# jjery2243542/adaptive_voice_conversion

Hardware: AMD Instinct MI355X
Metric: mel-segments/sec (80x128) train step (higher is better)
Workload: dtype f32; 1 GPU; BASELINE configs[1]: recon+KL train step (fwd, loss, bwd, clip, Adam-amsgrad), 80-mel x 128-frame segments, batch 256/GPU, fp32; global_batch=256, parallelism=dp1, world_size=1

## Files before the change

adaptive_voice_conversion_amd/_lib.py:

```python
import ctypes
import os

_HERE = os.path.dirname(os.path.abspath(__file__))
LIB_PATH = os.path.join(_HERE, "csrc", "libavc_hip.so")
_lib = None

MAX_BLOCKS = 8
PLAN_INFERENCE, PLAN_SPEAKER_ONLY = 1, 2
GRADS_ALL, GRADS_DECODER, GRADS_ENCODERS, GRADS_SPEAKER, GRADS_CONTENT = 0, 1, 2, 3, 4


class EncoderCfg(ctypes.Structure):
    _fields_ = [(n, ctypes.c_int) for n in ("c_in", "c_h", "c_out", "kernel_size", "bank_size", "bank_scale", "c_bank",
                                            "n_conv_blocks", "n_dense_blocks")] + [("subsample", ctypes.c_int * MAX_BLOCKS), ("act", ctypes.c_int)]


class DecoderCfg(ctypes.Structure):
    _fields_ = [(n, ctypes.c_int) for n in ("c_in", "c_cond", "c_h", "c_out", "kernel_size", "n_conv_blocks")] + \
               [("upsample", ctypes.c_int * MAX_BLOCKS), ("act", ctypes.c_int)]


class ModelCfg(ctypes.Structure):
    _fields_ = [("spk", EncoderCfg), ("enc", EncoderCfg), ("dec", DecoderCfg)]


class ReluSite(ctypes.Structure):
    _fields_ = [(n, ctypes.c_int) for n in ("kind", "B", "C", "T")] + \
               [(n, ctypes.c_long) for n in ("act_off", "sb", "sc", "st", "y_off", "stat_off", "cond_off", "cond_sb", "storage")]


class Tuning(ctypes.Structure):
    _fields_ = [(n, ctypes.c_int) for n in ("struct_size", "single_stream", "dec_split_min", "conv_x3", "wgrad_x3", "dgrad_par", "bank_switch",
                                            "conv_ck5", "wgrad_batch", "wgrad_batch_wgs", "wgrad_target_wgs", "conv_ablation", "wgrad_ablation",
                                            "op_compute_dtype", "side_prio", "tile12_wgs")] + \
               [(n, ctypes.c_long) for n in ("wgrad_batch_units", "tile_thr11", "tile_thr21", "ck16_wgs", "ck32_wgs", "kg_wgs", "conv_min_lds", "in_pairs_nv", "bh_ck5", "wgrad_cw8", "dec_wgrad_flush", "dec_wgrad_wgs", "conv_walk", "conv_walk_min", "conv_in_fuse", "dbg_streams")]


PLAN_X3 = 4
PLAN_RAGGED = 8
PLAN_BF16S = 16
PLAN_CONTENT_ONLY, PLAN_DECODER_ONLY, PLAN_PART_GRADS = 32, 64, 128
PLAN_INPUT_GRADS = 256
FWD_WEIGHTS_PACKED = 1
PLAN_EMB_INPUT = 512
ERR_PAIR_SHAPE = -12
c_void_p, c_long, c_int, c_float = ctypes.c_void_p, ctypes.c_long, ctypes.c_int, ctypes.c_float


def make_tuning(lib, overrides=None):
    t = Tuning()
# ... 140 lines not shown
```

adaptive_voice_conversion_amd/csrc/avc_common.h:

```cpp
#pragma once
#include <stdint.h>

#define AVC_MAX_GROUPS 8
#define AVC_THREADS 256

typedef float f32x16 __attribute__((ext_vector_type(16)));
typedef float f32x4 __attribute__((ext_vector_type(4)));
typedef short avc_s16x4 __attribute__((ext_vector_type(4)));

enum {
    AVC_COMPUTE_F32 = 0,
    AVC_COMPUTE_BF16 = 1,
    AVC_COMPUTE_F32X3 = 2,
    AVC_COMPUTE_BF16S = 3,
};

enum {
    AVC_RES_NONE = 0,
    AVC_RES_IDENTITY = 1,
    AVC_RES_AVGPOOL2 = 2,
    AVC_RES_POOLT = 3,
    AVC_RES_UPT = 4,
    AVC_RES_UP2 = 5,
};
// ... 94 lines not shown

struct WgradArgs {
    ConvSrc x;
    ConvSrc dy;
    int B, Cin, Cout, Tin, Tout;
    int KS, padL, stride;
    int chunks_per_sample, total_chunks, Tc, spc;
    int bf16;
    int tiles;
    int grp;
    int grid;
    int chunk_cost;
    int slots;
    int tNB, tWCO, tCW;
    int cw8;
    int rows_per_src;
    long cost_begin;
    long cost_total;
    long slab_need, dbslab_need;
    float* slab;
    float* dbslab;
    float* dw;
    float* db;
    long dw_src_stride, db_src_stride;
};
#define AVC_WGRAD_MAXL 16
struct WgradBatch {
    int nlayers;
    int dbg;
    int lds_floats;
// ... 202 lines not shown
```

adaptive_voice_conversion_amd/csrc/avc_internal.h:

```cpp
#pragma once
#include <string.h>

#include "avc_common.h"
#include "avc_hip.h"

struct PackArgs {
    const float* src[12];
    int nsrc, rows_per_src;
    int Cout, Cin, KS;
    int dgrad, CK, nchunk, M, Mp;
    float* dst;
    int img;
    int mb;
};

const avc_tuning& avc_default_tuning();
avc_tuning& avc_op_tuning();
long avc_pack_total(const PackArgs& p);

int avc_conv_ck(const avc_tuning& tun, int KS);
int avc_conv_pick_tile(const avc_tuning& tun, int Mp, int B, int Tout, int ngroups, int Kred);
long avc_conv_num_wgs(int tile, int Mp, int B, int Tout, int ngroups);
int avc_conv_ck_for(const avc_tuning& tun, int KS, long wgs, int mode, int stride, int Tout, int tile);
int avc_launch_conv(const ConvArgs& a, hipStream_t stream, int force_tile, const avc_tuning& tun);
// ... 13 lines not shown
int avc_launch_dsp_mag(const float* spec, int F, int T, float* mag, hipStream_t s);
int avc_launch_dsp_db_norm(const float* in, int C, int T, float ref_db, float max_db, float* out, hipStream_t s);
int avc_launch_dsp_denorm_amp(const float* in, int C, int T, float ref_db, float max_db, float* out, hipStream_t s);
int avc_launch_dsp_preemph(const float* y, long L, float a, float* out, hipStream_t s);
int avc_launch_dsp_deemph(const float* x, long L, float a, float* out, hipStream_t s);
int avc_launch_dsp_frame_power(const float* y, long L, int frame_length, int hop, int n_frames, float* out, hipStream_t s);
#define AVC_PACK_BATCH 16
int avc_launch_pack_batch(const PackArgs* ps, int n, hipStream_t stream);
#define AVC_PACK_PIECE 2048
#define AVC_PACK_STAGE 8192
int avc_pack_stage_rows(const PackArgs& p);
long avc_pack_pieces(const PackArgs& p);
int avc_launch_pack_table(const PackArgs* dev_tab, const void* dev_blk, int nblk, double bytes, const float* params, float* ws, hipStream_t stream);

void avc_wgrad_geometry(WgradArgs& a);
void avc_wgrad_plan_batch(WgradArgs* layers, int n, int target_wgs);
int avc_launch_wgrad_batch(const WgradArgs* layers, int n, hipStream_t stream, int ablation = 0);

int avc_launch_in_fwd(const INFwdArgs& a, hipStream_t s);
int avc_launch_in_bwd(const INBwdArgs& a, hipStream_t s);
int avc_launch_in_fwd_pairs(const INFwdArgs& a, hipStream_t s);
int avc_launch_in_bwd_pairs(const INBwdArgs& a, hipStream_t s);
int avc_launch_to_pairs(const float* x, long sxb, long sxc, long sxt, int B, int C, int T, float* dst, long db, long dc, hipStream_t s);
int avc_launch_reparam_fwd_pairs(const float* muls, const float* eps, int B, int C, int Tb, float* z, hipStream_t s);
int avc_launch_timepool_fwd_pairs(const float* in, int B, int C, int T, float* out, hipStream_t s);
int avc_launch_timepool_bwd_pairs(const float* dP, const float* amask, int B, int C, int T, float* G, float* dy, float slope, hipStream_t s);
int avc_launch_rag_in_fwd(const RagINArgs& a, hipStream_t s);
int avc_launch_rag_copy_rows(const float* x, long xsc, long xst, const int* T, const int* off, int B, int M, int sumT, float* dst, int CC, int c0,
                             hipStream_t s);
int avc_launch_rag_timepool_fwd(const float* in, const int* T, const int* off, int B, int C, float* out, hipStream_t s);
// ... 47 lines not shown
```

adaptive_voice_conversion_amd/csrc/conv_wgrad.hip:

```cpp
#include <hip/hip_runtime.h>
#include <stdlib.h>
#include <string.h>
#include <type_traits>
#include <vector>

#include "avc_common.h"
#include "avc_internal.h"
#include "conv_x3_shared.h"
#include "bf16_pairs.h"

static constexpr __host__ __device__ int wg_dyrow(bool lin) { return lin ? 36 : 33; }
static constexpr __host__ __device__ int wg_xrow_lin(int KS) {
    int r = (31 + KS + 3) / 4;
    return 4 * (r | 1);
}
#define WG_THREADS 512
static constexpr __host__ __device__ int wg_threads(int CW) { return (CW + 4) * 64; }

static constexpr __host__ __device__ int wg_group(int BF, int NB) { return BF == 2 ? (NB >= 4 ? 2 : 4) : 1; }
static constexpr __host__ __device__ int wg_stages(int BF, int NB) { return 2 * wg_group(BF, NB); }
#ifndef AVC_WGRAD_BHX_WAVES
#define AVC_WGRAD_BHX_WAVES 3
#endif

// ... 46 lines not shown
        const int cc = a.chunk_cost;
        s.layer = layer;
        s.tile = (int)(g / a.total_chunks);
        s.c_begin = (int)(g - (long)s.tile * a.total_chunks);
        const long tile_last = (long)(s.tile + 1) * a.total_chunks;
        s.c_end = (int)((g_end < tile_last ? g_end : tile_last) - (long)s.tile * a.total_chunks);
        g += s.c_end - s.c_begin;
        const long cs = a.cost_begin + (long)s.tile * a.total_chunks * cc;
        const int w_first = (int)((cs * G) / Ctot), w_last = (int)(((cs + (long)(a.total_chunks - 1) * cc) * G) / Ctot);
        s.nsplit = w_last - w_first + 1;
        s.z = w - w_first;
        return true;
    }
};

template <int KS, bool RT, int NB, int WCO, bool LIN, int BF, int CW = 4>
struct WgCfg {
    static constexpr int WCI = CW / WCO;
    static constexpr int TCO = 32 * WCO;
    static constexpr int TCI = 32 * NB * WCI;
    static constexpr int NACC = KS * NB;
    static constexpr bool BH = BF == 2;
    static constexpr int RCO = BH ? TCO / 2 : TCO, RCI = BH ? TCI / 2 : TCI;
    static constexpr int WG_DYROW = wg_dyrow(LIN);
    static constexpr int NPD = (RCO * WG_DYROW + 255) / 256;
    static constexpr int NPX = (RCI * (LIN ? wg_xrow_lin(KS) : (KS == 1 ? 33 : 71)) + 255) / 256;
    static constexpr int TPR = 256 / RCO;
    static constexpr int CPT = 32 / TPR;
    static constexpr int NBROW = BH ? 16 : 32;
    static constexpr int GRP = wg_group(BF, NB);
    static constexpr int NSTG = wg_stages(BF, NB);
    static constexpr bool BHX = BH && LIN && !RT;
    static constexpr int ROW16 = 40;
    static constexpr int ND16 = (RCO * 10 + 63) / 64, NX16 = (RCI * 10 + 63) / 64;
    static constexpr int NPD16 = (ND16 + 3) / 4, NPX16 = (NX16 + 3) / 4;
};
static __device__ __forceinline__ bool wg_wide16(const WgradArgs& a) {
    return (a.Tout & 31) == 0 && a.Tin == a.Tout && a.spc == 1 && a.x.st == 1 && a.dy.st == 1 && a.x.ps == 1 && a.dy.ps == 1 &&
           ((a.x.sc | a.x.sb | a.dy.sc | a.dy.sb) & 3) == 0 && ((((unsigned long)a.x.ptr) | ((unsigned long)a.dy.ptr)) & 15) == 0;
}

template <int KS, bool RT, int NB, int WCO, bool LIN, int BF, int CW>
static __device__ __forceinline__ void wg_producer(const WgradBatch& bt, float* smem, int tid, int lane, int wave) {
    using C = WgCfg<KS, RT, NB, WCO, LIN, BF, CW>;
    constexpr int TCO = C::TCO, TCI = C::TCI, RCO = C::RCO, RCI = C::RCI, WG_DYROW = C::WG_DYROW, NPD = C::NPD, NPX = C::NPX, TPR = C::TPR, CPT = C::CPT;
    constexpr int NSTG = C::NSTG, GRP = C::GRP;
    constexpr bool BH = C::BH;
    const int dbg = bt.dbg;
    const int ptid = tid & 255;
    unsigned dyo[NPD], xo[NPX];
    int xq[NPX];
    WgSegIter it(bt);
    WgSeg sg;
    while (it.next(bt, sg)) {
        const WgradArgs& a = bt.L[sg.layer];
        const int KSr = RT ? a.KS : KS;
        const int ci_tiles = avc_cdiv(a.Cin, TCI);
        const int CoutR = BH ? a.Cout >> 1 : a.Cout, CinR = BH ? a.Cin >> 1 : a.Cin;
        const float* xptr = a.x.ptr;
        const float* dyptr = a.dy.ptr;
        const int Tc = a.Tc, spc = a.spc;
        const int lgTc = 31 - __builtin_clz(Tc);
        const int XSEG = (Tc - 1) * a.stride + KSr;
        const int XROW = LIN ? wg_xrow_lin(KSr) : ((spc * XSEG) | 1);
        const bool wide = C::BHX && wg_wide16(a);
        const int DYROWW = wide ? C::ROW16 : WG_DYROW;
        const int DYS = wide ? RCO * C::ROW16 : RCO * WG_DYROW, XS = wide ? RCI * C::ROW16 : RCI * XROW;
        const int DYSP = wide ? (DYS + 255) & ~255 : (DYS + 63) & ~63, XSP = wide ? (XS + 255) & ~255 : (XS + 63) & ~63;
        float* dyT = smem;
        float* xT = smem + NSTG * DYSP;
        const float inv_xrow = 1.0f / (float)XROW;
        const int tile = sg.tile, c_begin = sg.c_begin, c_end = sg.c_end;
        const int co0 = (tile / ci_tiles) * TCO, ci0 = (tile % ci_tiles) * TCI;
        const int co0r = BH ? co0 >> 1 : co0, ci0r = BH ? ci0 >> 1 : ci0;
        const bool do_db = (a.db != nullptr) && (ci0 == 0);
        float dbsum = 0.f, dbsum1 = 0.f;
        const bool fastm = !wide && (spc > 1) && (a.Tout == Tc) && (a.B % spc == 0) && (XSP <= NPX * 256);
        const bool fastp = wide || fastm || ((spc == 1) && (a.Tout % 32 == 0) && (XSP <= NPX * 256));
        unsigned dyo16[C::BHX ? C::NPD16 : 1], xo16[C::BHX ? C::NPX16 : 1];
        int xedge[C::BHX ? C::NPX16 : 1];
        if constexpr (C::BHX) {
            if (wide) {
#pragma unroll
                for (int i = 0; i < C::NPD16; ++i) {
                    const int f = (wave + 4 * i) * 64 + lane;
                    int row = f / 10;
                    const int pc = f - row * 10;
                    row = row < RCO ? row : RCO - 1;
                    int co = co0r + row;
                    co = co < CoutR ? co : CoutR - 1;
                    dyo16[i] = 4u * (unsigned)((long)co * a.dy.sc + 4 * (pc < 8 ? pc : 0));
                }
#pragma unroll
                for (int i = 0; i < C::NPX16; ++i) {
                    const int f = (wave + 4 * i) * 64 + lane;
                    int row = f / 10;
                    const int pc = f - row * 10;
                    row = row < RCI ? row : RCI - 1;
                    int ci = ci0r + row;
                    ci = ci < CinR ? ci : CinR - 1;
                    xo16[i] = 4u * (unsigned)((long)ci * a.x.sc + 4 * pc);
                    xedge[i] = pc == 0 ? 1 : (pc == 9 ? -1 : 0);
                }
            }
        }
        auto issue16 = [&](int chunk, int buf) {
            if constexpr (C::BHX) {
                const int cb = chunk / a.chunks_per_sample;
                const int t0 = (chunk - cb * a.chunks_per_sample) * 32;
                const float* dyb = dyptr + ((long)cb * a.dy.sb + t0);
                const float* xb = xptr + ((long)cb * a.x.sb + t0) - 4;
                const bool first = t0 == 0, last = t0 + 32 == a.Tout;
                float* dd = dyT + buf * DYSP;
                float* xd = xT + buf * XSP;
#pragma unroll
                for (int i = 0; i < C::NPD16; ++i)
                    if (wave + 4 * i < C::ND16) avc_glds16_s(dyb, dyo16[i], dd + (wave + 4 * i) * 256);
#pragma unroll
                for (int i = 0; i < C::NPX16; ++i)
                    if (wave + 4 * i < C::NX16) {
                        unsigned v = xo16[i];
                        if (first && xedge[i] > 0) v += 16u;
                        if (last && xedge[i] < 0) v -= 16u;
                        avc_glds16_s(xb, v, xd + (wave + 4 * i) * 256);
                    }
            }
// ... 174 lines not shown
                    a.db[(long)(co / rows) * a.db_src_stride + co % rows] = v0;
                    a.db[(long)((co + 1) / rows) * a.db_src_stride + (co + 1) % rows] = v1;
                }
            } else {
                const int co = co0 + ptid / TPR;
                if (co < a.Cout) a.db[(long)(co / rows) * a.db_src_stride + co % rows] = v0;
            }
        };
        if (do_db) {
#pragma unroll
            for (int o = 1; o < TPR; o <<= 1) {
                dbsum += __shfl_xor(dbsum, o);
                if (BH) dbsum1 += __shfl_xor(dbsum1, o);
            }
        }
        if (dbg & 8) continue;
        if (sg.nsplit == 1) {
            if (do_db) store_db(dbsum, dbsum1);
            continue;
        }
        float* dbs_t = do_db ? a.dbslab + ((long)(tile / ci_tiles) * a.slots) * TCO : nullptr;
        if (do_db && (ptid % TPR) == 0) {
            if constexpr (BH) {
                dbs_t[(long)sg.z * TCO + 2 * (ptid / TPR)] = dbsum;
                dbs_t[(long)sg.z * TCO + 2 * (ptid / TPR) + 1] = dbsum1;
            } else {
                dbs_t[(long)sg.z * TCO + ptid / TPR] = dbsum;
            }
        }
    }
}

template <int KS, bool RT, int NB, int WCO, bool LIN, int BF, bool X3, int CW>
static __device__ __forceinline__ void wg_consumer(const WgradBatch& bt, float* smem, int tid, int lane, int wave) {
    using C = WgCfg<KS, RT, NB, WCO, LIN, BF, CW>;
    constexpr int WCI = C::WCI, TCO = C::TCO, TCI = C::TCI, NACC = C::NACC, RCO = C::RCO, RCI = C::RCI, WG_DYROW = C::WG_DYROW, NBROW = C::NBROW;
    constexpr int NSTG = C::NSTG;
    constexpr bool BH = C::BH;
    const int dbg = bt.dbg;
    const int wave_m = wave / WCI, wave_n = wave % WCI, li = lane & 31, h = lane >> 5;
    f32x16 acc[NACC];
    WgSegIter it(bt);
    WgSeg sg;
    while (it.next(bt, sg)) {
        const WgradArgs& a = bt.L[sg.layer];
        const int KSr = RT ? a.KS : KS;
        const int ci_tiles = avc_cdiv(a.Cin, TCI);
        const int Tc = a.Tc, spc = a.spc;
        const int lgTc = 31 - __builtin_clz(Tc);
        const int XSEG = (Tc - 1) * a.stride + KSr;
        const int XROW = LIN ? wg_xrow_lin(KSr) : ((spc * XSEG) | 1);
        const bool wide = C::BHX && wg_wide16(a);
        const int DYS = wide ? RCO * C::ROW16 : RCO * WG_DYROW, XS = wide ? RCI * C::ROW16 : RCI * XROW;
        const int DYSP = wide ? (DYS + 255) & ~255 : (DYS + 63) & ~63, XSP = wide ? (XS + 255) & ~255 : (XS + 63) & ~63;
        const float* dyT = smem;
        const float* xT = smem + NSTG * DYSP;
        int tcs = wide ? sg.c_begin % a.chunks_per_sample : 0;
        const long tile_floats = (long)CW * KSr * NB * 1024;
        const int tile = sg.tile, c_begin = sg.c_begin, c_end = sg.c_end;
        const int co0 = (tile / ci_tiles) * TCO, ci0 = (tile % ci_tiles) * TCI;
#pragma unroll
        for (int j = 0; j < NACC; ++j)
#pragma unroll
            for (int r = 0; r < 16; ++r) acc[j][r] = 0.f;
        __syncthreads();
        __syncthreads();
        auto chunk_loop = [&](auto wtag) {
        constexpr bool WIDE = decltype(wtag)::value;
        constexpr int GRP = C::GRP;
        for (int chunk = c_begin; chunk < c_end; ++chunk) {
            const int rel = chunk - c_begin;
            const int buf = GRP == 1 ? (rel & 1) : ((rel / GRP) & 1) * GRP + rel % GRP;
            const bool first_c = tcs == 0, last_c = tcs == a.chunks_per_sample - 1;
            if (WIDE && ++tcs == a.chunks_per_sample) tcs = 0;
            if (!(dbg & 2)) {
                const float* arow = dyT + buf * DYSP + (BH ? (wave_m * 32 + li) >> 1 : wave_m * 32 + li) * (WIDE ? C::ROW16 : WG_DYROW);
                const float* brow = xT + buf * XSP + (BH ? (wave_n * NB * 32 + li) >> 1 : wave_n * NB * 32 + li) * (WIDE ? C::ROW16 : XROW);
                auto body = [&](auto ktag) {
                    constexpr int K = decltype(ktag)::value;
                    auto tap_on = [&](int j) { return !RT || j < KSr; };
                    const float* arow_h = arow + h;
                    const float* brow_h = brow + h;
                    auto ldfrag = [&](int s, float& av, float (&bv)[NB * K]) {
                        const float* bp;
                        if constexpr (LIN) {
                            av = arow_h[2 * s];
                            bp = brow_h + 2 * s;
                        } else {
                            const int qcol = 2 * s + h;
                            const int sl = qcol >> lgTc, tl = qcol & (Tc - 1);
                            av = arow[qcol];
                            bp = brow + sl * XSEG + tl * a.stride;
// ... 11 lines not shown
                                constexpr int PADL = K / 2, PADR = (K & 1) ? K / 2 : K / 2 - 1;
                                constexpr int P0 = (4 - PADL) / 4, P1 = (11 + PADR) / 4;
                                auto fetchw = [&](int kb, unsigned (&ad)[8], unsigned (&xr)[NB][16]) {
                                    const float* ap = arow + 16 * kb + 8 * h;
                                    const float* bp = brow + 16 * kb + 8 * h;
#pragma unroll
                                    for (int i4 = 0; i4 < 2; ++i4) {
                                        const f32x4 v = *(const f32x4*)(ap + 4 * i4);
#pragma unroll
                                        for (int i = 0; i < 4; ++i) ad[4 * i4 + i] = bh_as_u32(v[i]);
                                    }
#pragma unroll
                                    for (int nb = 0; nb < NB; ++nb)
#pragma unroll
                                        for (int i4 = P0; i4 <= P1; ++i4) {
                                            const f32x4 v = *(const f32x4*)(bp + nb * NBROW * C::ROW16 + 4 * i4);
#pragma unroll
                                            for (int i = 0; i < 4; ++i) xr[nb][4 * i4 + i] = bh_as_u32(v[i]);
                                        }
                                };
                                auto blockw = [&](int kb, const unsigned (&ad)[8], unsigned (&xr)[NB][16]) {
                                    if (PADL > 0 && first_c && kb == 0) {
#pragma unroll
                                        for (int nb = 0; nb < NB; ++nb)
#pragma unroll
                                            for (int i = 1; i <= PADL; ++i) xr[nb][4 - i] = h == 0 ? xr[nb][4 + i] : xr[nb][4 - i];
                                    }
                                    if (PADR > 0 && last_c && kb == 1) {
#pragma unroll
                                        for (int nb = 0; nb < NB; ++nb)
#pragma unroll
// ... 128 lines not shown
                                    f32x16& c = acc[nb * KS + j];
                                    c = avc_mfma_bf16x8(at[2], q0, c);
                                    c = avc_mfma_bf16x8(at[0], q2, c);
                                    c = avc_mfma_bf16x8(at[1], q1, c);
                                    c = avc_mfma_bf16x8(at[1], q0, c);
                                    c = avc_mfma_bf16x8(at[0], q1, c);
                                    c = avc_mfma_bf16x8(at[0], q0, c);
                                }
                            }
                        };
                        float a0[8], x0[NB][NX], a1[8], x1[NB][NX];
                        fetch(0, a0, x0);
                        fetch(1, a1, x1);
                        block(a0, x0);
                        block(a1, x1);
                    } else if constexpr (LIN) {
                        constexpr int NX4 = (K + 6) / 4;
                        auto ldgrp = [&](int gq, f32x4& av, f32x4 (&xv)[NB][NX4]) {
                            const int c = 8 * gq + 4 * h;
                            av = *(const f32x4*)(arow + c);
#pragma unroll
                            for (int nb = 0; nb < NB; ++nb)
#pragma unroll
                                for (int i4 = 0; i4 < NX4; ++i4)
                                    if (!RT || 4 * i4 < 3 + KSr) xv[nb][i4] = *(const f32x4*)(brow + nb * 32 * XROW + c + 4 * i4);
                        };
                        f32x4 av[2], xv[2][NB][NX4];
                        ldgrp(0, av[0], xv[0]);
#pragma unroll
                        for (int gq = 0; gq < 4; ++gq) {
                            const int cur = gq & 1;
                            if (gq + 1 < 4) ldgrp(gq + 1, av[cur ^ 1], xv[cur ^ 1]);
                            __builtin_amdgcn_sched_barrier(0);
                            if constexpr (BF != 0) {
                                const avc_s16x4 ap = avc_pack_bf16x4(av[cur][0], av[cur][1], av[cur][2], av[cur][3]);
#pragma unroll
                                for (int nb = 0; nb < NB; ++nb)
#pragma unroll
                                    for (int j = 0; j < K; ++j) {
                                        if (!tap_on(j)) continue;
// ... 46 lines not shown
#pragma unroll
                            for (int nb = 0; nb < NB; ++nb)
#pragma unroll
                                for (int j = 0; j < K; ++j)
                                    if (tap_on(j)) acc[nb * KS + j] = __builtin_amdgcn_mfma_f32_32x32x2f32(av[cur], bv[cur][nb * K + j], acc[nb * KS + j], 0, 0, 0);
                            __builtin_amdgcn_sched_barrier(0);
                        }
                    }
                };
                static_assert(!RT || KS == 8, "run-time tap counts are built for up to 8 taps");
                body(KTag<KS>{});
            }
            if (!(dbg & 4) && (GRP == 1 || rel % GRP == GRP - 1 || chunk + 1 == c_end)) __syncthreads();
        }
        };
        if constexpr (C::BHX) {
            if (wide) chunk_loop(std::true_type{});
            else chunk_loop(std::false_type{});
        } else {
            chunk_loop(std::false_type{});
        }

        auto store_final = [&]() {
            const int rows = a.rows_per_src;
#pragma unroll
            for (int nb = 0; nb < NB; ++nb) {
                const int ci = ci0 + (wave_n * NB + nb) * 32 + li;
#pragma unroll
                for (int r = 0; r < 16; ++r) {
                    const int co = co0 + wave_m * 32 + (r & 3) + 8 * (r >> 2) + 4 * h;
                    if (co < a.Cout && ci < a.Cin) {
// ... 63 lines not shown

struct WgradKey {
    int KST, rt, NB, WCO, CW, lin;
    bool operator==(const WgradKey& o) const { return KST == o.KST && rt == o.rt && NB == o.NB && WCO == o.WCO && CW == o.CW && lin == o.lin; }
};
static size_t wgrad_lds_bytes_for(const WgradArgs& a, int NB, int WCO, int CW) {
    const int half = a.bf16 == AVC_COMPUTE_BF16S ? 2 : 1;
    const int TCO = 32 * WCO / half, TCI = 32 * NB * (CW / WCO) / half;
    const int XSEG = (a.Tc - 1) * a.stride + a.KS;
    const bool lin = a.Tc == 32 && a.stride == 1;
    const int XROW = lin ? wg_xrow_lin(a.KS) : ((a.spc * XSEG) | 1), WG_DYROW = wg_dyrow(lin);
    size_t stage = (size_t)((TCO * WG_DYROW + 63) & ~63) + ((TCI * XROW + 63) & ~63);
    if (half == 2 && lin) {
        const size_t s16 = (size_t)((TCO * 40 + 255) & ~255) + ((TCI * 40 + 255) & ~255);
        stage = s16 > stage ? s16 : stage;
    }
    return (size_t)wg_stages(half == 2 ? 2 : 0, NB) * stage * 4 + 64;
}
static WgradKey wgrad_key(const WgradArgs& a) {
    WgradKey k;
    wgrad_shape(a, &k.NB, &k.WCO, &k.CW);
    if (a.KS == 1 && k.NB == 4 && wgrad_lds_bytes_for(a, 4, 4, 4) > 158 * 1024) {
        k.NB = 1;
        k.WCO = 2;
    }
    if (k.CW == 8 && wgrad_lds_bytes_for(a, k.NB, k.WCO, 8) > 158 * 1024) {
        k.CW = 4;
        k.WCO = 2;
    }
    if (a.KS == 1) { k.KST = 1; k.rt = 0; }
    else if (a.KS == 5 && (k.WCO == 2 || k.CW == 8)) { k.KST = 5; k.rt = 0; }
    else { k.KST = 8; k.rt = 1; }
    k.lin = (a.Tc == 32 && a.stride == 1) ? 1 : 0;
    return k;
}

void avc_wgrad_geometry(WgradArgs& a) {
    if (a.Tout >= 32) {
        a.Tc = 32;
        a.spc = 1;
        a.chunks_per_sample = avc_cdiv(a.Tout, 32);
        a.total_chunks = a.B * a.chunks_per_sample;
    } else {
        int p = 1;
        while (p < a.Tout) p <<= 1;
        a.Tc = p;
        a.spc = 32 / p;
        a.chunks_per_sample = 1;
        a.total_chunks = avc_cdiv(a.B, a.spc);
// ... 276 lines not shown
```

adaptive_voice_conversion_amd/csrc/engine.hip:

```cpp
#include <hip/hip_runtime.h>
#include <math.h>
#include <stdio.h>
#include <stdlib.h>

#include <algorithm>
#include <map>
#include <string>
#include <vector>

#include "avc_common.h"
#include "avc_hip.h"
#include "avc_internal.h"

static thread_local std::string g_err;
static int fail(int rc, const char* what) {
    char buf[256];
    snprintf(buf, sizeof(buf), "%s (rc=%d)", what, rc);
    g_err = buf;
    return rc;
}
#define RUN(expr)                                  \
    do {                                           \
        int _rc = (expr);                          \
        if (_rc != 0) return fail(_rc, #expr);     \
// ... 932 lines not shown
    if (c.dry) return 0;
    return avc_launch_wgrad_batch(L.data(), n, ls, c.p->tun.wgrad_ablation);
}

static int wgrad_layer(BwdCtx& c, const LayerP& L, const float* x, long xsb, long xsc, int xst, const float* dy, long ysb,
                       long ysc, int yst, int yps, int Bn, int Tin, int Tout) {
    BwdCtx::PendW pw;
    WgradArgs& a = pw.a;
    memset(&a, 0, sizeof(a));
    a.x.ptr = x; a.x.sb = xsb; a.x.sc = xsc; a.x.st = xst; a.x.ps = 1;
    a.dy.ptr = dy; a.dy.sb = ysb; a.dy.sc = ysc; a.dy.st = yst; a.dy.ps = yps;
    a.B = Bn; a.Cin = L.Cin; a.Cout = L.Cout; a.Tin = Tin; a.Tout = Tout;
    a.KS = L.KS; a.padL = L.KS / 2; a.stride = L.stride;
    a.bf16 = (L.bf16 == AVC_COMPUTE_F32 && c.p->tun.wgrad_x3) ? AVC_COMPUTE_F32X3 : L.bf16;
    a.cw8 = c.p->tun.wgrad_cw8 ? 1 : 0;
    pw.L = &L;
    avc_wgrad_geometry(a);
    c.pend_units += (long)a.tiles * a.total_chunks;
    c.pend.push_back(pw);
    if (!c.hold && ((int)c.pend.size() >= c.p->tun.wgrad_batch || c.pend_units >= c.p->tun.wgrad_batch_units)) return flush_wgrads(c);
    return 0;
}

static void pack_layer(const avc_plan* p, const LayerP& L, const float* params, float* ws, std::vector<PackArgs>& out) {
    PackArgs a;
    memset(&a, 0, sizeof(a));
    for (int i = 0; i < L.nsrc; ++i) a.src[i] = p->par(params, L.w[i]);
    a.src[0] += L.src_off;
    a.nsrc = L.nsrc; a.rows_per_src = L.rows;
    a.Cout = L.Cout; a.Cin = L.Cin; a.KS = L.KS;
// ... 1375 lines not shown
```

adaptive_voice_conversion_amd/csrc/ops_api.hip:

```cpp
#include <hip/hip_runtime.h>
#include <math.h>

#include "avc_common.h"
#include "avc_internal.h"

#include <string.h>

static avc_tuning make_default_tuning() {
    avc_tuning t;
    memset(&t, 0, sizeof(t));
    t.struct_size = (int)sizeof(avc_tuning);
    t.dec_split_min = 128;
    t.dgrad_par = 1;
    t.side_prio = 1;
    t.bank_switch = 1;
    t.conv_ck5 = 8;
    t.wgrad_batch = 12;
    t.wgrad_batch_wgs = 256;
    t.wgrad_target_wgs = 256;
    t.wgrad_batch_units = 1L << 40;
    t.tile_thr11 = 8192;
    t.tile_thr21 = 4096;
    t.ck16_wgs = 256;
    t.ck32_wgs = 256;
    t.kg_wgs = 256;
    t.bh_ck5 = 8;
    t.in_pairs_nv = 1;
    t.wgrad_cw8 = 0;
    t.dec_wgrad_flush = 0;
    t.dec_wgrad_wgs = 128;
    t.conv_walk = 0;
    t.conv_walk_min = 2;
    t.conv_in_fuse = 1;
    return t;
}
const avc_tuning& avc_default_tuning() {
    static const avc_tuning t = make_default_tuning();
    return t;
}
avc_tuning& avc_op_tuning() {
    static thread_local avc_tuning t = make_default_tuning();
    return t;
}

extern "C" {
void avc_tuning_init(avc_tuning* t) {
    if (t) *t = avc_default_tuning();
}
void avc_get_op_tuning(avc_tuning* out) {
    if (out) *out = avc_op_tuning();
}
int avc_set_tuning(const char* name, int value) {
    if (!name) return -1;
    avc_tuning& t = avc_op_tuning();
#define AVC_TUNE_FIELD(f) if (!strcmp(name, #f)) { t.f = value; return 0; }
    AVC_TUNE_FIELD(single_stream) AVC_TUNE_FIELD(dec_split_min) AVC_TUNE_FIELD(conv_x3) AVC_TUNE_FIELD(wgrad_x3) AVC_TUNE_FIELD(dgrad_par)
    AVC_TUNE_FIELD(bank_switch) AVC_TUNE_FIELD(conv_ck5) AVC_TUNE_FIELD(wgrad_batch) AVC_TUNE_FIELD(wgrad_batch_wgs) AVC_TUNE_FIELD(wgrad_target_wgs)
    AVC_TUNE_FIELD(conv_ablation) AVC_TUNE_FIELD(wgrad_ablation) AVC_TUNE_FIELD(op_compute_dtype) AVC_TUNE_FIELD(tile12_wgs) AVC_TUNE_FIELD(side_prio) AVC_TUNE_FIELD(wgrad_batch_units)
    AVC_TUNE_FIELD(tile_thr11) AVC_TUNE_FIELD(tile_thr21) AVC_TUNE_FIELD(ck16_wgs) AVC_TUNE_FIELD(ck32_wgs) AVC_TUNE_FIELD(kg_wgs) AVC_TUNE_FIELD(bh_ck5) AVC_TUNE_FIELD(in_pairs_nv) AVC_TUNE_FIELD(conv_min_lds) AVC_TUNE_FIELD(wgrad_cw8) AVC_TUNE_FIELD(dec_wgrad_flush) AVC_TUNE_FIELD(dec_wgrad_wgs)
    AVC_TUNE_FIELD(conv_walk) AVC_TUNE_FIELD(conv_walk_min) AVC_TUNE_FIELD(conv_in_fuse) AVC_TUNE_FIELD(dbg_streams)
#undef AVC_TUNE_FIELD
    if (!strcmp(name, "compute")) { t.op_compute_dtype = (value == AVC_COMPUTE_BF16) ? AVC_COMPUTE_BF16 : AVC_COMPUTE_F32; return 0; }
    return -1;
}

long avc_packed_weight_floats_x3(int Cout, int Cin, int KS, int dgrad) {
    const int Cred = dgrad ? Cout : Cin;
    if (!((KS == 5 && Cred % 16 == 0) || (KS == 1 && Cred >= 32))) return -1;
    return avc_conv_x3_image_floats(dgrad ? Cin : Cout, Cred, KS);
}
int avc_pack_weight_x3(const float* w, int Cout, int Cin, int KS, int dgrad, float* dst, void* stream) {
    if (avc_packed_weight_floats_x3(Cout, Cin, KS, dgrad) < 0) return -2;
    PackArgs p;
    avc_pack_x3_args(p, w, Cout, Cin, KS, dgrad, dst);
    return avc_launch_pack(p, (hipStream_t)stream);
// ... 141 lines not shown
    a.g[0].wp = wpd; a.g[0].bias = nullptr; a.g[0].out = dx; a.g[0].out2 = dx2; a.g[0].res = res; a.g[0].mask = mask;
    a.g[0].KS = KS; a.g[0].padL = padL; a.g[0].padR = padR; a.g[0].nchunk = avc_cdiv(a.Cred, a.g[0].CK);
    a.img = bh ? AVC_IMG_K4H : AVC_IMG_K4;
    if (tile == 97) { a.img = AVC_IMG_X3; a.g[0].CK = KS == 1 ? 32 : 16; a.g[0].nchunk = avc_cdiv(Cout, a.g[0].CK); }
    return avc_launch_conv(a, (hipStream_t)stream, tile, avc_op_tuning());
}

static void op_wgrad_args(WgradArgs& a, int B, int Cin, int Cout, int Tin, int Tout, int KS, int stride) {
    memset(&a, 0, sizeof(a));
    const avc_tuning& t = avc_op_tuning();
    a.bf16 = (t.op_compute_dtype == AVC_COMPUTE_F32 && t.wgrad_x3) ? AVC_COMPUTE_F32X3 : (op_bh() ? AVC_COMPUTE_BF16S : t.op_compute_dtype);
    a.B = B; a.Cin = Cin; a.Cout = Cout; a.Tin = Tin; a.Tout = Tout;
    a.KS = KS; a.padL = KS / 2; a.stride = stride;
    a.x.ps = 1; a.dy.ps = 1;
    a.cw8 = t.wgrad_cw8 ? 1 : 0;
}
int avc_conv1d_dgrad_in_bwd(const float* dy, long syb, long syc, int syt, int yps, int B, int Cout, int Tdy, const float* wpd, int Cin, int KS,
                            int stride, int Tin, float* g_out, const float* res, int res_mode, int Tres, const float* y, const float* mean,
                            const float* rstd, const float* cond, long cond_sb, int cond_off, int relu, float* dy_out, float* dcond,
                            long dcond_sb, int dcond_off, int* fused, void* stream) {
    const bool bh = op_bh();
    if (bh && (avc_op_tuning().op_compute_dtype != AVC_COMPUTE_BF16S || (Cin & 1) || (Cout & 1))) return -2;
    ConvArgs a;
    memset(&a, 0, sizeof(a));
    op_compute(a);
    a.x.ptr = dy; a.x.sb = syb; a.x.sc = syc; a.x.st = syt; a.x.ps = yps;
    a.B = B; a.Cred = bh ? Cout / 2 : Cout; a.Tsrc = Tdy;
    a.mode = 1; a.stride = stride;
    const int padL = KS / 2, padR = (KS % 2 == 0) ? KS / 2 - 1 : KS / 2;
    a.mirror = (KS > 1) ? 1 : 0;
// ... 13 lines not shown
    if (fused) *fused = fuse ? 1 : 0;
    if (fuse) {
        a.inb.dy = dy_out; a.inb.y = y; a.inb.mean = mean; a.inb.rstd = rstd;
        a.inb.cond = cond; a.inb.cond_sb = cond_sb; a.inb.cond_off = cond_off;
        a.inb.dcond = dcond; a.inb.dcond_sb = dcond_sb; a.inb.dcond_off = dcond_off;
        a.inb.C = Cin; a.inb.relu = relu ? 1 : 0;
        return avc_launch_conv(a, (hipStream_t)stream, 0, avc_op_tuning());
    }
    if (!g_out) return -1;
    int rc = avc_launch_conv(a, (hipStream_t)stream, 0, avc_op_tuning());
    if (rc) return rc;
    if (bh) return avc_instnorm_bwd_pairs(g_out, y, mean, rstd, B, Cin, Tin, cond, cond_sb, cond_off, relu, 0, dy_out, dcond, dcond_sb, dcond_off, stream);
    return avc_instnorm_bwd(g_out, y, mean, rstd, B, Cin, Tin, cond, cond_sb, cond_off, relu, dy_out, dcond, dcond_sb, dcond_off, stream);
}

long avc_conv1d_wgrad_ws_floats(int B, int Cin, int Cout, int Tout, int KS) {
    long need = 0;
    for (int stride = 1; stride <= 2; ++stride) {
        WgradArgs a;
        op_wgrad_args(a, B, Cin, Cout, Tout * stride, Tout, KS, stride);
        avc_wgrad_plan_batch(&a, 1, avc_op_tuning().wgrad_target_wgs);
        const long n = a.slab_need + a.dbslab_need + 64;
        need = n > need ? n : need;
    }
    return need;
}
int avc_conv1d_wgrad(const float* x, long sxb, long sxc, int sxt, const float* dy, long syb, long syc, int syt, int yps,
                     int B, int Cin, int Cout, int Tin, int Tout, int KS, int stride, float* dW, float* db, float* ws,
                     void* stream) {
    WgradArgs a;
// ... 83 lines not shown
```

include/avc_hip.h:

```cpp
#ifndef AVC_HIP_H
#define AVC_HIP_H
#ifdef __cplusplus
extern "C" {
#endif

#define AVC_MAX_BLOCKS 8

typedef struct avc_encoder_cfg {
    int c_in, c_h, c_out, kernel_size, bank_size, bank_scale, c_bank, n_conv_blocks, n_dense_blocks;
    int subsample[AVC_MAX_BLOCKS];
    int act;
} avc_encoder_cfg;

typedef struct avc_decoder_cfg {
    int c_in, c_cond, c_h, c_out, kernel_size, n_conv_blocks;
    int upsample[AVC_MAX_BLOCKS];
    int act;
} avc_decoder_cfg;

typedef struct avc_model_cfg {
    avc_encoder_cfg spk;
    avc_encoder_cfg enc;
    avc_decoder_cfg dec;
} avc_model_cfg;
// ... 56 lines not shown
    int op_compute_dtype;
    int side_prio;
    int tile12_wgs;
    long wgrad_batch_units;
    long tile_thr11, tile_thr21, ck16_wgs, ck32_wgs, kg_wgs;
    long conv_min_lds;
    long in_pairs_nv;
    long bh_ck5;
    long wgrad_cw8;
    long dec_wgrad_flush;
    long dec_wgrad_wgs;
    long conv_walk;
    long conv_walk_min;
    long conv_in_fuse;
    long dbg_streams;
} avc_tuning;
void avc_tuning_init(avc_tuning* t);
#define AVC_PLAN_X3 4
#define AVC_PLAN_RAGGED 8
#define AVC_PLAN_BF16S 16
#define AVC_ERR_PAIR_SHAPE (-12)
int avc_plan_create_tuned(const avc_model_cfg* cfg, int B, int T, int T_cond, int flags, const avc_tuning* tuning, avc_plan** out);
int avc_plan_set_single_stream(avc_plan* p, int on);

int avc_plan_set_compute_dtype(avc_plan* p, int dtype);
int avc_plan_compute_dtype(const avc_plan* p);

int avc_forward(const avc_plan* p, const float* params, const float* x, long sxb, long sxc, int sxt,
                const float* x_cond, long scb, long scc, int sct, const float* eps, float* ws, void* stream);
#define AVC_FWD_WEIGHTS_PACKED 1
// ... 71 lines not shown
                    float* dst, void* stream);
long avc_packed_weight_floats_x3(int Cout, int Cin, int KS, int dgrad);
int avc_pack_weight_x3(const float* w, int Cout, int Cin, int KS, int dgrad, float* dst, void* stream);
int avc_conv1d_fwd(const float* x, long sxb, long sxc, int sxt, int B, int Cin, int Tin, const float* wp,
                   const float* bias, int Cout, int KS, int stride, int act, float* out, long ob, long oc, int ot,
                   int ops, const float* res, int res_mode, long rb, long rc, int rt, int Tres, float* out2, int tile,
                   void* stream);
int avc_conv1d_dgrad(const float* dy, long syb, long syc, int syt, int yps, int B, int Cout, int Tdy, const float* wpd,
                     int Cin, int KS, int stride, int Tin, float* dx, long ob, long oc, int ot, const float* res,
                     int res_mode, long rb, long rc, int rt, int Tres, float* dx2, const float* mask, int tile,
                     void* stream);
long avc_conv1d_wgrad_ws_floats(int B, int Cin, int Cout, int Tout, int KS);
int avc_conv1d_wgrad(const float* x, long sxb, long sxc, int sxt, const float* dy, long syb, long syc, int syt, int yps,
                     int B, int Cin, int Cout, int Tin, int Tout, int KS, int stride, float* dW, float* db, float* ws,
                     void* stream);
int avc_instnorm_fwd(const float* y, int B, int C, int T, const float* cond, long cond_sb, int cond_off, int relu,
                     const float* res, int res_mode, int Tres, float* out, float* mean, float* rstd, void* stream);
int avc_instnorm_bwd(const float* g, const float* y, const float* mean, const float* rstd, int B, int C, int T,
                     const float* cond, long cond_sb, int cond_off, int relu, float* dy, float* dcond, long dcond_sb,
                     int dcond_off, void* stream);
int avc_conv1d_in_fwd(const float* x, long sxb, long sxc, int sxt, int B, int Cin, int Tin, const float* wp, const float* bias, int Cout, int KS,
                      int stride, int ops, float* y, const float* cond, long cond_sb, int cond_off, int relu, const float* res, int res_mode,
                      int Tres, float* out, float* mean, float* rstd, int* fused, void* stream);
int avc_conv1d_dgrad_in_bwd(const float* dy, long syb, long syc, int syt, int yps, int B, int Cout, int Tdy, const float* wpd, int Cin, int KS,
                            int stride, int Tin, float* g_out, const float* res, int res_mode, int Tres, const float* y, const float* mean,
                            const float* rstd, const float* cond, long cond_sb, int cond_off, int relu, float* dy_out, float* dcond,
                            long dcond_sb, int dcond_off, int* fused, void* stream);

#ifdef __cplusplus
}
// ... 3 lines not shown
```

Measured before the change: 43560 mel-segments/sec.

## Extend wide 16-byte staged wgrad loads to fp32 KS=5/KS=1 linear kernels

Lets the fp32 weight-gradient kernel for KS=5 and KS=1 linear layers use the wide 16-byte vectorized staging path (padded LDS rows), which was previously only available to the bf16-pair variant. The per-segment body becomes a lambda instantiated for wide and non-wide modes. A dedicated KS=5 MFMA inner loop is added that double-buffers A and X register loads and patches the sequence edges in registers. The feature is on by default through a new tuning knob, and it adds code size, register pressure and an LDS staging-size increase.

```diff
diff --git a/adaptive_voice_conversion_amd/_lib.py b/adaptive_voice_conversion_amd/_lib.py
--- a/adaptive_voice_conversion_amd/_lib.py
+++ b/adaptive_voice_conversion_amd/_lib.py
@@ -33,7 +33,7 @@
     _fields_ = [(n, ctypes.c_int) for n in ("struct_size", "single_stream", "dec_split_min", "conv_x3", "wgrad_x3", "dgrad_par", "bank_switch",
                                             "conv_ck5", "wgrad_batch", "wgrad_batch_wgs", "wgrad_target_wgs", "conv_ablation", "wgrad_ablation",
                                             "op_compute_dtype", "side_prio", "tile12_wgs")] + \
-               [(n, ctypes.c_long) for n in ("wgrad_batch_units", "tile_thr11", "tile_thr21", "ck16_wgs", "ck32_wgs", "kg_wgs", "conv_min_lds", "in_pairs_nv", "bh_ck5", "wgrad_cw8", "dec_wgrad_flush", "dec_wgrad_wgs", "conv_walk", "conv_walk_min", "conv_in_fuse", "dbg_streams")]
+               [(n, ctypes.c_long) for n in ("wgrad_batch_units", "tile_thr11", "tile_thr21", "ck16_wgs", "ck32_wgs", "kg_wgs", "conv_min_lds", "in_pairs_nv", "bh_ck5", "wgrad_cw8", "dec_wgrad_flush", "dec_wgrad_wgs", "conv_walk", "conv_walk_min", "conv_in_fuse", "dbg_streams", "wgrad_stage16")]
 
 
 PLAN_X3 = 4
diff --git a/adaptive_voice_conversion_amd/csrc/avc_common.h b/adaptive_voice_conversion_amd/csrc/avc_common.h
--- a/adaptive_voice_conversion_amd/csrc/avc_common.h
+++ b/adaptive_voice_conversion_amd/csrc/avc_common.h
@@ -132,6 +132,7 @@
     int slots;
     int tNB, tWCO, tCW;
     int cw8;
+    int st16;
     int rows_per_src;
     long cost_begin;
     long cost_total;
diff --git a/adaptive_voice_conversion_amd/csrc/avc_internal.h b/adaptive_voice_conversion_amd/csrc/avc_internal.h
--- a/adaptive_voice_conversion_amd/csrc/avc_internal.h
+++ b/adaptive_voice_conversion_amd/csrc/avc_internal.h
@@ -51,6 +51,7 @@
 int avc_launch_pack_table(const PackArgs* dev_tab, const void* dev_blk, int nblk, double bytes, const float* params, float* ws, hipStream_t stream);
 
 void avc_wgrad_geometry(WgradArgs& a);
+bool avc_wgrad_stage16(const WgradArgs& a);
 void avc_wgrad_plan_batch(WgradArgs* layers, int n, int target_wgs);
 int avc_launch_wgrad_batch(const WgradArgs* layers, int n, hipStream_t stream, int ablation = 0);
 
diff --git a/adaptive_voice_conversion_amd/csrc/conv_wgrad.hip b/adaptive_voice_conversion_amd/csrc/conv_wgrad.hip
--- a/adaptive_voice_conversion_amd/csrc/conv_wgrad.hip
+++ b/adaptive_voice_conversion_amd/csrc/conv_wgrad.hip
@@ -84,6 +84,9 @@
     }
 };
 
+static constexpr __host__ __device__ bool wg_f32_stage16(int KS, bool RT, bool LIN, int BF, int CW) {
+    return BF == 0 && LIN && !RT && CW == 4 && (KS == 5 || KS == 1);
+}
 template <int KS, bool RT, int NB, int WCO, bool LIN, int BF, int CW = 4>
 struct WgCfg {
     static constexpr int WCI = CW / WCO;
@@ -101,13 +104,19 @@
     static constexpr int GRP = wg_group(BF, NB);
     static constexpr int NSTG = wg_stages(BF, NB);
     static constexpr bool BHX = BH && LIN && !RT;
-    static constexpr int ROW16 = 40;
-    static constexpr int ND16 = (RCO * 10 + 63) / 64, NX16 = (RCI * 10 + 63) / 64;
+    static constexpr bool F16 = wg_f32_stage16(KS, RT, LIN, BF, CW);
+    static constexpr bool W16 = BHX || F16;
+    static constexpr int PD16 = BH ? 10 : 9, PX16 = BH ? 10 : (KS == 5 ? 11 : 9);
+    static constexpr int PDV = 8, PXV = BH ? 10 : (KS == 5 ? 10 : 8);
+    static constexpr int XLEAD = BH ? 4 : (KS == 5 ? 4 : 0);
+    static constexpr int ROWD16 = 4 * PD16, ROWX16 = 4 * PX16;
+    static constexpr int ND16 = (RCO * PD16 + 63) / 64, NX16 = (RCI * PX16 + 63) / 64;
     static constexpr int NPD16 = (ND16 + 3) / 4, NPX16 = (NX16 + 3) / 4;
 };
-static __device__ __forceinline__ bool wg_wide16(const WgradArgs& a) {
-    return (a.Tout & 31) == 0 && a.Tin == a.Tout && a.spc == 1 && a.x.st == 1 && a.dy.st == 1 && a.x.ps == 1 && a.dy.ps == 1 &&
-           ((a.x.sc | a.x.sb | a.dy.sc | a.dy.sb) & 3) == 0 && ((((unsigned long)a.x.ptr) | ((unsigned long)a.dy.ptr)) & 15) == 0;
+static __host__ __device__ inline bool wg_wide16(const WgradArgs& a, bool pair) {
+    return (pair || (a.st16 && a.bf16 == AVC_COMPUTE_F32)) && (a.Tout & 31) == 0 && a.Tin == a.Tout && a.spc == 1 && a.stride == 1 && a.x.st == 1 &&
+           a.dy.st == 1 && a.x.ps == 1 && a.dy.ps == 1 && ((a.x.sc | a.x.sb | a.dy.sc | a.dy.sb) & 3) == 0 &&
+           ((((unsigned long)a.x.ptr) | ((unsigned long)a.dy.ptr)) & 15) == 0;
 }
 
 template <int KS, bool RT, int NB, int WCO, bool LIN, int BF, int CW>
@@ -118,11 +127,12 @@
     constexpr bool BH = C::BH;
     const int dbg = bt.dbg;
     const int ptid = tid & 255;
-    unsigned dyo[NPD], xo[NPX];
-    int xq[NPX];
     WgSegIter it(bt);
     WgSeg sg;
-    while (it.next(bt, sg)) {
+    auto segment = [&](auto wtag) {
+        constexpr int WM = decltype(wtag)::value;
+        unsigned dyo[NPD], xo[NPX];
+        int xq[NPX];
         const WgradArgs& a = bt.L[sg.layer];
         const int KSr = RT ? a.KS : KS;
         const int ci_tiles = avc_cdiv(a.Cin, TCI);
@@ -133,9 +143,9 @@
         const int lgTc = 31 - __builtin_clz(Tc);
         const int XSEG = (Tc - 1) * a.stride + KSr;
         const int XROW = LIN ? wg_xrow_lin(KSr) : ((spc * XSEG) | 1);
-        const bool wide = C::BHX && wg_wide16(a);
-        const int DYROWW = wide ? C::ROW16 : WG_DYROW;
-        const int DYS = wide ? RCO * C::ROW16 : RCO * WG_DYROW, XS = wide ? RCI * C::ROW16 : RCI * XROW;
+        const bool wide = WM == 2 ? (C::W16 && wg_wide16(a, BH)) : WM == 1;
+        const int DYROWW = wide ? C::ROWD16 : WG_DYROW;
+        const int DYS = wide ? RCO * C::ROWD16 : RCO * WG_DYROW, XS = wide ? RCI * C::ROWX16 : RCI * XROW;
         const int DYSP = wide ? (DYS + 255) & ~255 : (DYS + 63) & ~63, XSP = wide ? (XS + 255) & ~255 : (XS + 63) & ~63;
         float* dyT = smem;
         float* xT = smem + NSTG * DYSP;
@@ -147,39 +157,39 @@
         float dbsum = 0.f, dbsum1 = 0.f;
         const bool fastm = !wide && (spc > 1) && (a.Tout == Tc) && (a.B % spc == 0) && (XSP <= NPX * 256);
         const bool fastp = wide || fastm || ((spc == 1) && (a.Tout % 32 == 0) && (XSP <= NPX * 256));
-        unsigned dyo16[C::BHX ? C::NPD16 : 1], xo16[C::BHX ? C::NPX16 : 1];
-        int xedge[C::BHX ? C::NPX16 : 1];
-        if constexpr (C::BHX) {
+        unsigned dyo16[C::W16 ? C::NPD16 : 1], xo16[C::W16 ? C::NPX16 : 1];
+        int xedge[C::W16 ? C::NPX16 : 1];
+        if constexpr (C::W16) {
             if (wide) {
 #pragma unroll
                 for (int i = 0; i < C::NPD16; ++i) {
                     const int f = (wave + 4 * i) * 64 + lane;
-                    int row = f / 10;
-                    const int pc = f - row * 10;
+                    int row = f / C::PD16;
+                    const int pc = f - row * C::PD16;
                     row = row < RCO ? row : RCO - 1;
                     int co = co0r + row;
                     co = co < CoutR ? co : CoutR - 1;
-                    dyo16[i] = 4u * (unsigned)((long)co * a.dy.sc + 4 * (pc < 8 ? pc : 0));
+                    dyo16[i] = 4u * (unsigned)((long)co * a.dy.sc + 4 * (pc < C::PDV ? pc : 0));
                 }
 #pragma unroll
                 for (int i = 0; i < C::NPX16; ++i) {
                     const int f = (wave + 4 * i) * 64 + lane;
-                    int row = f / 10;
-                    const int pc = f - row * 10;
+                    int row = f / C::PX16;
+                    const int pc = f - row * C::PX16;
                     row = row < RCI ? row : RCI - 1;
                     int ci = ci0r + row;
                     ci = ci < CinR ? ci : CinR - 1;
-                    xo16[i] = 4u * (unsigned)((long)ci * a.x.sc + 4 * pc);
-                    xedge[i] = pc == 0 ? 1 : (pc == 9 ? -1 : 0);
+                    xo16[i] = 4u * (unsigned)((long)ci * a.x.sc + 4 * (pc < C::PXV ? pc : C::XLEAD / 4));
+                    xedge[i] = C::XLEAD == 0 ? 0 : (pc == 0 ? 1 : (pc == 9 ? -1 : 0));
                 }
             }
         }
         auto issue16 = [&](int chunk, int buf) {
-            if constexpr (C::BHX) {
+            if constexpr (C::W16) {
                 const int cb = chunk / a.chunks_per_sample;
                 const int t0 = (chunk - cb * a.chunks_per_sample) * 32;
                 const float* dyb = dyptr + ((long)cb * a.dy.sb + t0);
-                const float* xb = xptr + ((long)cb * a.x.sb + t0) - 4;
+                const float* xb = xptr + ((long)cb * a.x.sb + t0) - C::XLEAD;
                 const bool first = t0 == 0, last = t0 + 32 == a.Tout;
                 float* dd = dyT + buf * DYSP;
                 float* xd = xT + buf * XSP;
@@ -384,10 +394,10 @@
                 if (BH) dbsum1 += __shfl_xor(dbsum1, o);
             }
         }
-        if (dbg & 8) continue;
+        if (dbg & 8) return;
         if (sg.nsplit == 1) {
             if (do_db) store_db(dbsum, dbsum1);
-            continue;
+            return;
         }
         float* dbs_t = do_db ? a.dbslab + ((long)(tile / ci_tiles) * a.slots) * TCO : nullptr;
         if (do_db && (ptid % TPR) == 0) {
@@ -397,6 +407,14 @@
             } else {
                 dbs_t[(long)sg.z * TCO + ptid / TPR] = dbsum;
             }
+        }
+    };
+    while (it.next(bt, sg)) {
+        if constexpr (C::F16) {
+            if (wg_wide16(bt.L[sg.layer], false)) segment(KTag<1>{});
+            else segment(KTag<0>{});
+        } else {
+            segment(KTag<2>{});
         }
     }
 }
@@ -420,8 +438,9 @@
         const int lgTc = 31 - __builtin_clz(Tc);
         const int XSEG = (Tc - 1) * a.stride + KSr;
         const int XROW = LIN ? wg_xrow_lin(KSr) : ((spc * XSEG) | 1);
-        const bool wide = C::BHX && wg_wide16(a);
-        const int DYS = wide ? RCO * C::ROW16 : RCO * WG_DYROW, XS = wide ? RCI * C::ROW16 : RCI * XROW;
+        constexpr bool W16 = C::W16 && !X3;
+        const bool wide = W16 && wg_wide16(a, BH);
+        const int DYS = wide ? RCO * C::ROWD16 : RCO * WG_DYROW, XS = wide ? RCI * C::ROWX16 : RCI * XROW;
         const int DYSP = wide ? (DYS + 255) & ~255 : (DYS + 63) & ~63, XSP = wide ? (XS + 255) & ~255 : (XS + 63) & ~63;
         const float* dyT = smem;
         const float* xT = smem + NSTG * DYSP;
@@ -444,8 +463,8 @@
             const bool first_c = tcs == 0, last_c = tcs == a.chunks_per_sample - 1;
             if (WIDE && ++tcs == a.chunks_per_sample) tcs = 0;
             if (!(dbg & 2)) {
-                const float* arow = dyT + buf * DYSP + (BH ? (wave_m * 32 + li) >> 1 : wave_m * 32 + li) * (WIDE ? C::ROW16 : WG_DYROW);
-                const float* brow = xT + buf * XSP + (BH ? (wave_n * NB * 32 + li) >> 1 : wave_n * NB * 32 + li) * (WIDE ? C::ROW16 : XROW);
+                const float* arow = dyT + buf * DYSP + (BH ? (wave_m * 32 + li) >> 1 : wave_m * 32 + li) * (WIDE ? C::ROWD16 : WG_DYROW);
+                const float* brow = xT + buf * XSP + (BH ? (wave_n * NB * 32 + li) >> 1 : wave_n * NB * 32 + li) * (WIDE ? C::ROWX16 : XROW);
                 auto body = [&](auto ktag) {
                     constexpr int K = decltype(ktag)::value;
                     auto tap_on = [&](int j) { return !RT || j < KSr; };
@@ -487,7 +506,7 @@
                                     for (int nb = 0; nb < NB; ++nb)
 #pragma unroll
                                         for (int i4 = P0; i4 <= P1; ++i4) {
-                                            const f32x4 v = *(const f32x4*)(bp + nb * NBROW * C::ROW16 + 4 * i4);
+                                            const f32x4 v = *(const f32x4*)(bp + nb * NBROW * C::ROWX16 + 4 * i4);
 #pragma unroll
                                             for (int i = 0; i < 4; ++i) xr[nb][4 * i4 + i] = bh_as_u32(v[i]);
                                         }
@@ -646,6 +665,50 @@
                         fetch(1, a1, x1);
                         block(a0, x0);
                         block(a1, x1);
+                    } else if constexpr (LIN && WIDE && BF == 0 && K == 5) {
+                        constexpr int XR = C::ROWX16;
+                        f32x4 av[2], xp[NB][9];
+                        auto lda = [&](int gq, f32x4& a4) { a4 = *(const f32x4*)(arow + 8 * gq + 4 * h); };
+                        auto ldx = [&](int q) {
+#pragma unroll
+                            for (int nb = 0; nb < NB; ++nb) xp[nb][q] = *(const f32x4*)(brow + nb * 32 * XR + 4 * h + 4 * q);
+                        };
+                        lda(0, av[0]);
+                        ldx(0);
+                        ldx(1);
+                        ldx(2);
+#pragma unroll
+                        for (int gq = 0; gq < 4; ++gq) {
+                            const int cur = gq & 1;
+                            if (gq + 1 < 4) {
+                                lda(gq + 1, av[cur ^ 1]);
+                                ldx(2 * gq + 3);
+                                ldx(2 * gq + 4);
+                            }
+                            __builtin_amdgcn_sched_barrier(0);
+                            if (gq == 0 && first_c) {
+#pragma unroll
+                                for (int nb = 0; nb < NB; ++nb) {
+                                    xp[nb][0][3] = h == 0 ? xp[nb][1][1] : xp[nb][0][3];
+                                    xp[nb][0][2] = h == 0 ? xp[nb][1][2] : xp[nb][0][2];
+                                }
+                            }
+                            if (gq == 3 && last_c) {
+#pragma unroll
+                                for (int nb = 0; nb < NB; ++nb) {
+                                    xp[nb][8][0] = h == 1 ? xp[nb][7][2] : xp[nb][8][0];
+                                    xp[nb][8][1] = h == 1 ? xp[nb][7][1] : xp[nb][8][1];
+                                }
+                            }
+#pragma unroll
+                            for (int u = 0; u < 4; ++u)
+#pragma unroll
+                                for (int nb = 0; nb < NB; ++nb)
+#pragma unroll
+                                    for (int j = 0; j < K; ++j)
+                                        acc[nb * KS + j] = __builtin_amdgcn_mfma_f32_32x32x2f32(av[cur][u], xp[nb][2 * gq + ((u + j + 2) >> 2)][(u + j + 2) & 3], acc[nb * KS + j], 0, 0, 0);
+                            __builtin_amdgcn_sched_barrier(0);
+                        }
                     } else if constexpr (LIN) {
                         constexpr int NX4 = (K + 6) / 4;
                         auto ldgrp = [&](int gq, f32x4& av, f32x4 (&xv)[NB][NX4]) {
@@ -655,7 +718,7 @@
                             for (int nb = 0; nb < NB; ++nb)
 #pragma unroll
                                 for (int i4 = 0; i4 < NX4; ++i4)
-                                    if (!RT || 4 * i4 < 3 + KSr) xv[nb][i4] = *(const f32x4*)(brow + nb * 32 * XROW + c + 4 * i4);
+                                    if (!RT || 4 * i4 < 3 + KSr) xv[nb][i4] = *(const f32x4*)(brow + nb * 32 * (WIDE ? C::ROWX16 : XROW) + c + 4 * i4);
                         };
                         f32x4 av[2], xv[2][NB][NX4];
                         ldgrp(0, av[0], xv[0]);
@@ -732,7 +795,7 @@
             if (!(dbg & 4) && (GRP == 1 || rel % GRP == GRP - 1 || chunk + 1 == c_end)) __syncthreads();
         }
         };
-        if constexpr (C::BHX) {
+        if constexpr (W16) {
             if (wide) chunk_loop(std::true_type{});
             else chunk_loop(std::false_type{});
         } else {
@@ -826,6 +889,9 @@
     if (half == 2 && lin) {
         const size_t s16 = (size_t)((TCO * 40 + 255) & ~255) + ((TCI * 40 + 255) & ~255);
         stage = s16 > stage ? s16 : stage;
+    } else if (a.st16 && a.bf16 == AVC_COMPUTE_F32 && wg_f32_stage16(a.KS, a.KS == 5 && WCO != 2, lin, 0, CW)) {
+        const size_t s16 = (size_t)((TCO * 36 + 255) & ~255) + ((TCI * (a.KS == 5 ? 44 : 36) + 255) & ~255);
+        stage = s16 > stage ? s16 : stage;
     }
     return (size_t)wg_stages(half == 2 ? 2 : 0, NB) * stage * 4 + 64;
 }
@@ -845,6 +911,13 @@
     else { k.KST = 8; k.rt = 1; }
     k.lin = (a.Tc == 32 && a.stride == 1) ? 1 : 0;
     return k;
+}
+
+bool avc_wgrad_stage16(const WgradArgs& a) {
+    const WgradKey k = wgrad_key(a);
+    const bool pair = a.bf16 == AVC_COMPUTE_BF16S;
+    const bool inst = pair ? (k.lin && !k.rt) : wg_f32_stage16(k.KST, k.rt != 0, k.lin != 0, a.bf16 == AVC_COMPUTE_BF16 ? 1 : 0, k.CW);
+    return inst && wg_wide16(a, pair);
 }
 
 void avc_wgrad_geometry(WgradArgs& a) {
diff --git a/adaptive_voice_conversion_amd/csrc/engine.hip b/adaptive_voice_conversion_amd/csrc/engine.hip
--- a/adaptive_voice_conversion_amd/csrc/engine.hip
+++ b/adaptive_voice_conversion_amd/csrc/engine.hip
@@ -970,6 +970,7 @@
     a.KS = L.KS; a.padL = L.KS / 2; a.stride = L.stride;
     a.bf16 = (L.bf16 == AVC_COMPUTE_F32 && c.p->tun.wgrad_x3) ? AVC_COMPUTE_F32X3 : L.bf16;
     a.cw8 = c.p->tun.wgrad_cw8 ? 1 : 0;
+    a.st16 = c.p->tun.wgrad_stage16 ? 1 : 0;
     pw.L = &L;
     avc_wgrad_geometry(a);
     c.pend_units += (long)a.tiles * a.total_chunks;
diff --git a/adaptive_voice_conversion_amd/csrc/ops_api.hip b/adaptive_voice_conversion_amd/csrc/ops_api.hip
--- a/adaptive_voice_conversion_amd/csrc/ops_api.hip
+++ b/adaptive_voice_conversion_amd/csrc/ops_api.hip
@@ -32,6 +32,7 @@
     t.conv_walk = 0;
     t.conv_walk_min = 2;
     t.conv_in_fuse = 1;
+    t.wgrad_stage16 = 1;
     return t;
 }
 const avc_tuning& avc_default_tuning() {
@@ -58,7 +59,7 @@
     AVC_TUNE_FIELD(bank_switch) AVC_TUNE_FIELD(conv_ck5) AVC_TUNE_FIELD(wgrad_batch) AVC_TUNE_FIELD(wgrad_batch_wgs) AVC_TUNE_FIELD(wgrad_target_wgs)
     AVC_TUNE_FIELD(conv_ablation) AVC_TUNE_FIELD(wgrad_ablation) AVC_TUNE_FIELD(op_compute_dtype) AVC_TUNE_FIELD(tile12_wgs) AVC_TUNE_FIELD(side_prio) AVC_TUNE_FIELD(wgrad_batch_units)
     AVC_TUNE_FIELD(tile_thr11) AVC_TUNE_FIELD(tile_thr21) AVC_TUNE_FIELD(ck16_wgs) AVC_TUNE_FIELD(ck32_wgs) AVC_TUNE_FIELD(kg_wgs) AVC_TUNE_FIELD(bh_ck5) AVC_TUNE_FIELD(in_pairs_nv) AVC_TUNE_FIELD(conv_min_lds) AVC_TUNE_FIELD(wgrad_cw8) AVC_TUNE_FIELD(dec_wgrad_flush) AVC_TUNE_FIELD(dec_wgrad_wgs)
-    AVC_TUNE_FIELD(conv_walk) AVC_TUNE_FIELD(conv_walk_min) AVC_TUNE_FIELD(conv_in_fuse) AVC_TUNE_FIELD(dbg_streams)
+    AVC_TUNE_FIELD(conv_walk) AVC_TUNE_FIELD(conv_walk_min) AVC_TUNE_FIELD(conv_in_fuse) AVC_TUNE_FIELD(dbg_streams) AVC_TUNE_FIELD(wgrad_stage16)
 #undef AVC_TUNE_FIELD
     if (!strcmp(name, "compute")) { t.op_compute_dtype = (value == AVC_COMPUTE_BF16) ? AVC_COMPUTE_BF16 : AVC_COMPUTE_F32; return 0; }
     return -1;
@@ -230,6 +231,7 @@
     a.KS = KS; a.padL = KS / 2; a.stride = stride;
     a.x.ps = 1; a.dy.ps = 1;
     a.cw8 = t.wgrad_cw8 ? 1 : 0;
+    a.st16 = t.wgrad_stage16 ? 1 : 0;
 }
 int avc_conv1d_dgrad_in_bwd(const float* dy, long syb, long syc, int syt, int yps, int B, int Cout, int Tdy, const float* wpd, int Cin, int KS,
                             int stride, int Tin, float* g_out, const float* res, int res_mode, int Tres, const float* y, const float* mean,
@@ -273,6 +275,15 @@
     return avc_instnorm_bwd(g_out, y, mean, rstd, B, Cin, Tin, cond, cond_sb, cond_off, relu, dy_out, dcond, dcond_sb, dcond_off, stream);
 }
 
+int avc_conv1d_wgrad_stage16(const float* x, long sxb, long sxc, int sxt, const float* dy, long syb, long syc, int syt, int yps,
+                             int B, int Cin, int Cout, int Tin, int Tout, int KS, int stride) {
+    WgradArgs a;
+    op_wgrad_args(a, B, Cin, Cout, Tin, Tout, KS, stride);
+    a.x.ptr = x; a.x.sb = sxb; a.x.sc = sxc; a.x.st = sxt; a.x.ps = 1;
+    a.dy.ptr = dy; a.dy.sb = syb; a.dy.sc = syc; a.dy.st = syt; a.dy.ps = yps;
+    avc_wgrad_plan_batch(&a, 1, avc_op_tuning().wgrad_target_wgs);
+    return avc_wgrad_stage16(a) ? 1 : 0;
+}
 long avc_conv1d_wgrad_ws_floats(int B, int Cin, int Cout, int Tout, int KS) {
     long need = 0;
     for (int stride = 1; stride <= 2; ++stride) {
diff --git a/include/avc_hip.h b/include/avc_hip.h
--- a/include/avc_hip.h
+++ b/include/avc_hip.h
@@ -94,6 +94,7 @@
     long conv_walk_min;
     long conv_in_fuse;
     long dbg_streams;
+    long wgrad_stage16;
 } avc_tuning;
 void avc_tuning_init(avc_tuning* t);
 #define AVC_PLAN_X3 4
@@ -195,6 +196,8 @@
 int avc_conv1d_wgrad(const float* x, long sxb, long sxc, int sxt, const float* dy, long syb, long syc, int syt, int yps,
                      int B, int Cin, int Cout, int Tin, int Tout, int KS, int stride, float* dW, float* db, float* ws,
                      void* stream);
+int avc_conv1d_wgrad_stage16(const float* x, long sxb, long sxc, int sxt, const float* dy, long syb, long syc, int syt, int yps,
+                             int B, int Cin, int Cout, int Tin, int Tout, int KS, int stride);
 int avc_instnorm_fwd(const float* y, int B, int C, int T, const float* cond, long cond_sb, int cond_off, int relu,
                      const float* res, int res_mode, int Tres, float* out, float* mean, float* rstd, void* stream);
 int avc_instnorm_bwd(const float* g, const float* y, const float* mean, const float* rstd, int B, int C, int T,
```

Measured after the change: 43770 mel-segments/sec, median of 6. No clear change (+0.5%).
